# osheraz/IsaacGymInsertion

Hardware: AMD Instinct MI355X
Metric: PPO update steps/sec (4096 envs x 32 horizon) (higher is better)
Workload: dtype f32; 1 GPU; teacher PPO update, MLP actor-critic 404,501 params, 4096 envs x 32 horizon per GPU, 8 mini-epochs x 8 minibatches of 16384 (BASELINE configs[1]); envs_per_gpu=4096, horizon=32, optimizer_steps_per_update=64, parallelism=dp1, grad_allreduce=none

## Files before the change

isaacgyminsertion_amd/csrc/rowblock.h:

```cpp
#pragma once
#include <type_traits>

#include "dma_util.h"
#include "gemm_f32.h"

namespace igi {

constexpr int RB_KO = 128;
constexpr int RB_S = 64;
constexpr int RB_BR = 64;
constexpr int RB_Z_FLOATS = RB_BR * RB_KO;
constexpr int RB_X_FLOATS = RB_BR * RB_S;
constexpr int RB_STAGE = RB_Z_FLOATS + RB_X_FLOATS;
constexpr int RB_EPLD = 32 + 4;
constexpr int RB_PARK = 4 * 32 * RB_EPLD;
constexpr int RB_WPLD = RB_S + 4;
constexpr int RB_DLT = 64 + 4;
constexpr int RB_LATZ = 64 * 8 + 8 * 128 + 4 * 256 + 16 * RB_DLT;
constexpr int RB_LDS_FLOATS = 2 * RB_STAGE + RB_PARK;
constexpr int RB_LDS_FLOATS_LATZ = RB_LDS_FLOATS + RB_LATZ;
constexpr int RB_THREADS = 512;
static_assert(4 * 32 * RB_WPLD <= RB_STAGE, "the final weight-gradient tiles park in stage 0");
static_assert(2 * (32 * 66 + 32) <= RB_PARK, "the LOWX exchange uses the parking slices");

struct RbLevelArgs {
  const float* dZ = nullptr; int ldz = 0; long long sZ = 0;
  const float* W = nullptr; int ldw = 0; long long sW = 0;
  const float* X = nullptr; int ldx = 0; long long sX = 0;
  float* dX = nullptr; int lddx = 0; long long sdX = 0;
  float* dWp = nullptr; int ldwp = 0; long long sWpart = 0, sWnet = 0;
  float* dBp = nullptr; long long sBpart = 0, sBnet = 0;
  int rows = 0, IN = 0, nets = 1;
  int nslices = 0, ranges = 0, nblocks = 0;
  const float* lx_X = nullptr; int lx_ld = 0;
  float* lx_W = nullptr; int lx_ldw = 0; long long lx_sPart = 0;
  float* lx_B = nullptr; long long lx_bsPart = 0;
  const float* lz_parts = nullptr; int lz_tiles = 0; long long lz_tstride = 0;
  const float* lz_lat = nullptr; int lz_ldlat = 0;
  const float* lz_W3 = nullptr;
  float* lz_rec = nullptr; long long lz_srec = 0;
};

static inline int rb_level_ranges(int rows, int IN, int nets) {
  const int nslices = IN / RB_S, nblocks = rows / RB_BR;
  int r = 256 / (nets * nslices);
  if (r > nblocks) r = nblocks;
  return r < 1 ? 1 : r;
}

static inline bool rb_level_shape_ok(long long rows, int KO, int IN, int nets) {
  return KO == RB_KO && IN >= RB_S && (IN % RB_S) == 0 && IN <= 1024 && rows >= 4 * RB_BR && (rows % RB_BR) == 0 &&
         rows < (1 << 24) && nets >= 1 && nets <= 2 && !bf16_mode();
}

template <int MODE, int NETS>
__global__ __launch_bounds__(RB_THREADS) void k_rb_level(const RbLevelArgs a) {
  constexpr bool LOWX = MODE == 2 || MODE == 3, LATZ = MODE == 3;
  extern __shared__ __attribute__((aligned(1024))) float smem[];
  const int tid = threadIdx.x, lane = tid & 63, wave = __builtin_amdgcn_readfirstlane(tid >> 6);
  const int l31 = lane & 31, h = lane >> 5;

  const int total_ranges = NETS * a.ranges;
  int slice, gr;
  {
    const int bid = blockIdx.x;
    if ((total_ranges & 7) == 0) {
      const int x = bid & 7, p = bid >> 3;
      const int q = p / a.nslices;
      slice = p - q * a.nslices;
      gr = x * (total_ranges >> 3) + q;
    } else {
      gr = bid / a.nslices;
      slice = bid - gr * a.nslices;
    }
  }
  slice = __builtin_amdgcn_readfirstlane(slice);
  gr = __builtin_amdgcn_readfirstlane(gr);
  const int net = NETS == 1 ? 0 : __builtin_amdgcn_readfirstlane(gr / a.ranges), range = gr - net * a.ranges;
  const int b0 = __builtin_amdgcn_readfirstlane((int)((long long)range * a.nblocks / a.ranges));
  const int b1 = __builtin_amdgcn_readfirstlane((int)((long long)(range + 1) * a.nblocks / a.ranges));
  const int nb = b1 - b0;
  const int c0 = slice * RB_S;
  const float* dZ = a.dZ + net * a.sZ + (long long)b0 * RB_BR * a.ldz;
  const float* X = a.X + net * a.sX + (long long)b0 * RB_BR * a.ldx + c0;
  float* dX = a.dX + net * a.sdX + (long long)b0 * RB_BR * a.lddx + c0;
  const float* W = a.W + net * a.sW + c0;

  const bool dgrad_role = wave < 4;
  const int w4 = wave & 3;

  float* dlb = smem + 2 * RB_STAGE + RB_PARK;
  float* w3s = dlb + 64 * 8;
  float* lzx = w3s + 8 * 128;
  float* dlt = lzx + 4 * 256;
  typedef float f32x4m __attribute__((ext_vector_type(4)));
  f32x4m acc3[2] = {{0.f, 0.f, 0.f, 0.f}, {0.f, 0.f, 0.f, 0.f}};
  auto latz_head = [&](const float* zs_c, auto wg_c) __attribute__((always_inline)) {
    constexpr bool WG = decltype(wg_c)::value;
    float* zs = const_cast<float*>(zs_c);
    if constexpr (WG) {
      const int n = lane & 15, q = lane >> 4;
      const f32x4 av = *reinterpret_cast<const f32x4*>(dlt + n * RB_DLT + 16 * w4 + 4 * q);
#pragma unroll
      for (int t = 0; t < 4; ++t) {
        const int rr = 4 * q + t;
        const float* yr = zs + (16 * w4 + rr) * RB_KO + (n & 3);
#pragma unroll
        for (int jt = 0; jt < 2; ++jt) {
          const float bv = yr[4 * ((8 * slice + 4 * jt + (n >> 2)) ^ rr)];
          acc3[jt] = __builtin_amdgcn_mfma_f32_16x16x4f32(av[t], bv, acc3[jt], 0, 0, 0);
        }
      }
    }
    asm volatile("s_waitcnt lgkmcnt(0)" ::: "memory");
    __builtin_amdgcn_s_barrier();
    asm volatile("" ::: "memory");
    {
      const int cg = tid & 31, rg = tid >> 5;
      f32x4 wv[8];
#pragma unroll
      for (int k = 0; k < 8; ++k) wv[k] = *reinterpret_cast<const f32x4*>(w3s + k * 128 + 4 * cg);
      float* zp0 = zs + rg * RB_KO + 4 * (cg ^ rg);
#pragma unroll
      for (int i = 0; i < 4; ++i) {
        const int row = rg + 16 * i;
        const f32x4 d0 = *reinterpret_cast<const f32x4*>(dlb + row * 8), d1 = *reinterpret_cast<const f32x4*>(dlb + row * 8 + 4);
        f32x4* zp = reinterpret_cast<f32x4*>(zp0 + 16 * i * RB_KO);
        const f32x4 y = *zp;
        f32x4 sacc = {0.f, 0.f, 0.f, 0.f};
#pragma unroll
        for (int k = 0; k < 8; ++k) {
          const float dk = k < 4 ? d0[k & 3] : d1[k & 3];
#pragma unroll
          for (int j = 0; j < 4; ++j) sacc[j] = fmaf(dk, wv[k][j], sacc[j]);
        }
        f32x4 o;
#pragma unroll
        for (int j = 0; j < 4; ++j) o[j] = sacc[j] * (1.0f - y[j] * y[j]);
        *zp = o;
      }
    }
    asm volatile("s_waitcnt lgkmcnt(0)" ::: "memory");
    __builtin_amdgcn_s_barrier();
    asm volatile("" ::: "memory");
  };

  if (dgrad_role) {
    const int rt = w4 >> 1, ct = w4 & 1;
    __builtin_amdgcn_s_barrier();
    asm volatile("" ::: "memory");
    float wf[64];
    int zq[16];
    {
      const float* wp = smem + RB_STAGE + 4 * h * RB_S + 32 * ct + l31;
#pragma unroll
      for (int c = 0; c < 16; ++c)
#pragma unroll
        for (int j = 0; j < 4; ++j) wf[4 * c + j] = wp[(8 * c + j) * RB_S];
      const int m = 32 * rt + l31;
#pragma unroll
      for (int c = 0; c < 16; ++c) zq[c] = m * RB_KO + 4 * ((2 * c + h) ^ (m & 15));
      asm volatile("s_waitcnt lgkmcnt(0)" ::: "memory");
    }
    __builtin_amdgcn_s_barrier();
    asm volatile("" ::: "memory");
    float* park = smem + 2 * RB_STAGE + w4 * (32 * RB_EPLD);
    const int prow = lane >> 3, pc4 = lane & 7;
    unsigned lo = 4u * ((unsigned)prow * (unsigned)a.lddx + 4u * (unsigned)pc4);
    f32x16 acc_prev;
    float xv_prev[16];
#pragma unroll
    for (int r = 0; r < 16; ++r) { acc_prev[r] = 0.f; xv_prev[r] = 0.f; }
    f32x16 lxacc[2];
    float lxb = 0.f, pb0[16], pb1[16];
#pragma unroll
    for (int r = 0; r < 16; ++r) { lxacc[0][r] = 0.f; lxacc[1][r] = 0.f; pb0[r] = 0.f; pb1[r] = 0.f; }
    const float* lxbase = LOWX ? a.lx_X + ((long long)b0 * RB_BR + 32 * rt) * a.lx_ld : nullptr;
    unsigned lxo = 4u * ((unsigned)(4 * h) * (unsigned)a.lx_ld + (unsigned)l31);
    auto lx_load = [&](int bp, int r) {
      const char* q = reinterpret_cast<const char*>(uniform_ptr(lxbase + ((long long)bp * RB_BR + (r & 3) + 8 * (r >> 2)) * a.lx_ld));
      asm volatile("" : "+v"(lxo));
      pb0[r] = *reinterpret_cast<const float*>(q + lxo);
      pb1[r] = *reinterpret_cast<const float*>(q + lxo + 128);
    };
    float vprev[16];
#pragma unroll
    for (int r = 0; r < 16; ++r) vprev[r] = 0.f;
    auto epi_elem = [&](int bp, int r) {
      const float v = LOWX ? vprev[r] : acc_prev[r] * (1.0f - xv_prev[r] * xv_prev[r]);
      if (LOWX) {
        lxb += v;
        lxacc[0] = __builtin_amdgcn_mfma_f32_32x32x2f32(v, pb0[r], lxacc[0], 0, 0, 0);
        lxacc[1] = __builtin_amdgcn_mfma_f32_32x32x2f32(v, pb1[r], lxacc[1], 0, 0, 0);
      } else {
        park[((r & 3) + 8 * (r >> 2) + 4 * h) * RB_EPLD + l31] = v;
      }
    };
    f32x4 pv;
    auto epi_read = [&](int it) { pv = *reinterpret_cast<const f32x4*>(park + (8 * it + prow) * RB_EPLD + 4 * pc4); };
    auto epi_store = [&](int bp, int it) {
      char* ob = reinterpret_cast<char*>(dX + ((long long)bp * RB_BR + 32 * rt) * a.lddx + 32 * ct);
      asm volatile("" : "+v"(lo));
      *reinterpret_cast<f32x4*>(ob + (size_t)it * 8 * a.lddx * 4 + lo) = pv;
    };
    auto block = [&](int b, auto stg) {
      constexpr int S = decltype(stg)::value;
      if (b > 0) {
        __builtin_amdgcn_s_barrier();
        asm volatile("" ::: "memory");
      }
      const float* zs = smem + S * RB_STAGE;
      const float* xs = zs + RB_Z_FLOATS;
      if constexpr (LATZ) latz_head(zs, std::false_type{});
      const float* xc = xs + (32 * rt + 4 * h) * RB_S + 32 * ct + l31;
      float xv[16];
      if (!LOWX) {
#pragma unroll
        for (int r = 0; r < 16; ++r) xv[r] = xc[((r & 3) + 8 * (r >> 2)) * RB_S];
      }
      f32x16 acc;
#pragma unroll
      for (int r = 0; r < 16; ++r) acc[r] = 0.f;
      f32x4 fa[2];
      const int zrow = (32 * rt + l31) * RB_KO, zsw = (32 * rt + l31) & 15;
      auto zoffs = [&](int c) { return LOWX ? zrow + 4 * ((2 * c + h) ^ zsw) : zq[c]; };
      fa[0] = *reinterpret_cast<const f32x4*>(zs + zoffs(0));
      const bool epi = b > 0;
      if (LOWX && epi) { lx_load(b - 1, 0); lx_load(b - 1, 1); }
#pragma unroll
      for (int c = 0; c < 16; ++c) {
        if (c < 15) fa[(c + 1) & 1] = *reinterpret_cast<const f32x4*>(zs + zoffs(c + 1));
        if (epi && MODE == 0 && c >= 9 && c < 13) epi_read(c - 9);
        __builtin_amdgcn_sched_barrier(0);
#pragma unroll
        for (int j = 0; j < 4; ++j)
          acc = __builtin_amdgcn_mfma_f32_32x32x2f32(fa[c & 1][j], wf[4 * c + j], acc, 0, 0, 0);
        if (epi) {
          if (LOWX) { if (c + 2 < 16) lx_load(b - 1, c + 2); epi_elem(b - 1, c); }
          else if (c < 8) { epi_elem(b - 1, 2 * c); epi_elem(b - 1, 2 * c + 1); }
          else if (c >= 9 && c < 13) epi_store(b - 1, c - 9);
        }
        __builtin_amdgcn_sched_barrier(0);
      }
      if (LOWX) {
#pragma unroll
        for (int r = 0; r < 16; ++r) xv[r] = xc[((r & 3) + 8 * (r >> 2)) * RB_S];
#pragma unroll
        for (int r = 0; r < 16; ++r) vprev[r] = acc[r] * (1.0f - xv[r] * xv[r]);
      } else {
        acc_prev = acc;
#pragma unroll
        for (int r = 0; r < 16; ++r) xv_prev[r] = xv[r];
      }
    };
    int b = 0;
    for (; b + 2 <= nb; b += 2) {
      block(b, std::integral_constant<int, 0>{});
      block(b + 1, std::integral_constant<int, 1>{});
    }
    if (b < nb) block(b, std::integral_constant<int, 0>{});
    __syncthreads();
    if constexpr (LATZ) {
      float* rec = a.lz_rec + (long long)range * a.lz_srec;
      float s3 = 0.f;
#pragma unroll
      for (int g = 0; g < 4; ++g) s3 += lzx[g * 256 + tid];
      rec[(tid >> 5) * 128 + 32 * slice + (tid & 31)] = s3;
      if (slice == 0 && tid < 8) {
        float sdb = 0.f;
        for (int j = 0; j < 32; ++j) sdb += dlb[tid + 8 * j];
        rec[8 * 128 + tid] = sdb;
      }
    }
    if (LOWX) { lx_load(nb - 1, 0); lx_load(nb - 1, 1); }
#pragma unroll
    for (int r = 0; r < 16; ++r) {
      if (LOWX && r + 2 < 16) lx_load(nb - 1, r + 2);
      epi_elem(nb - 1, r);
    }
    if (MODE == 0) {
#pragma unroll
      for (int it = 0; it < 4; ++it) { epi_read(it); epi_store(nb - 1, it); }
    }
    if (LOWX) {
      constexpr int XLD = 64 + 2;
      float* ex = smem + 2 * RB_STAGE + ct * (32 * XLD + 32);
      const float bsum2 = lxb + __shfl_xor(lxb, 32, 64);
      if (rt == 1) {
#pragma unroll
        for (int n = 0; n < 2; ++n)
#pragma unroll
          for (int r = 0; r < 16; ++r) ex[((r & 3) + 8 * (r >> 2) + 4 * h) * XLD + 32 * n + l31] = lxacc[n][r];
        if (h == 0) ex[32 * XLD + l31] = bsum2;
      }
      __syncthreads();
      if (rt == 0) {
        float* wout = a.lx_W + range * a.lx_sPart + (long long)(c0 + 32 * ct) * a.lx_ldw;
#pragma unroll
        for (int n = 0; n < 2; ++n)
#pragma unroll
          for (int r = 0; r < 16; ++r) {
            const int c = (r & 3) + 8 * (r >> 2) + 4 * h;
            wout[(long long)c * a.lx_ldw + 32 * n + l31] = lxacc[n][r] + ex[c * XLD + 32 * n + l31];
          }
        if (h == 0) a.lx_B[range * a.lx_bsPart + c0 + 32 * ct + l31] = bsum2 + ex[32 * XLD + l31];
      }
    }
    return;
  }

  const int zr0 = 2 * w4 + (lane >> 5);
  unsigned zoff[2];
#pragma unroll
  for (int par = 0; par < 2; ++par)
    zoff[par] = 4u * ((unsigned)zr0 * (unsigned)a.ldz + 4u * (unsigned)((lane & 31) ^ ((zr0 + 8 * par) & 15)));
  unsigned xoff = 4u * ((unsigned)(4 * w4 + (lane >> 4)) * (unsigned)a.ldx + 4u * (unsigned)(lane & 15));
  auto issue = [&](int b, auto stg) {
    float* st = smem + decltype(stg)::value * RB_STAGE;
    const char* zb = reinterpret_cast<const char*>(uniform_ptr(dZ + (long long)b * RB_BR * a.ldz));
    const char* xb = reinterpret_cast<const char*>(uniform_ptr(X + (long long)b * RB_BR * a.ldx));
#pragma unroll
    for (int q = 0; q < 8; ++q) {
      asm volatile("" : "+v"(zoff[q & 1]));
      dma16(reinterpret_cast<const float*>(zb + (size_t)q * 8 * a.ldz * 4 + zoff[q & 1]), st + 256 * (w4 + 4 * q));
    }
#pragma unroll
    for (int q = 0; q < 4; ++q) {
      asm volatile("" : "+v"(xoff));
      dma16(reinterpret_cast<const float*>(xb + (size_t)q * 16 * a.ldx * 4 + xoff), st + RB_Z_FLOATS + 256 * (w4 + 4 * q));
    }
  };
  issue(0, std::integral_constant<int, 0>{});
  {
    const unsigned woff = 4u * ((unsigned)(4 * w4 + (lane >> 4)) * (unsigned)a.ldw + 4u * (unsigned)(lane & 15));
    const char* wb = reinterpret_cast<const char*>(uniform_ptr(W));
#pragma unroll
    for (int q = 0; q < 8; ++q)
      dma16(reinterpret_cast<const float*>(wb + (size_t)q * 16 * a.ldw * 4 + woff), smem + RB_STAGE + 256 * (w4 + 4 * q));
  }
  const int wt = tid - 256;
  float lzp[2][8], lzl[2] = {0.f, 0.f};
  float dbacc = 0.f;
#pragma unroll
  for (int i = 0; i < 2; ++i)
#pragma unroll
    for (int t = 0; t < 8; ++t) lzp[i][t] = 0.f;
  auto lz_fetch = [&](int b) __attribute__((always_inline)) {
#pragma unroll
    for (int i = 0; i < 2; ++i) {
      const int pr = wt + 256 * i;
      const long long grow = (long long)(b0 + b) * RB_BR + (pr >> 3);
      const float* pp = a.lz_parts + grow * 8 + (pr & 7);
#pragma unroll
      for (int t = 0; t < 8; ++t) lzp[i][t] = t < a.lz_tiles ? pp[(long long)t * a.lz_tstride] : 0.f;
      lzl[i] = a.lz_lat[grow * a.lz_ldlat + (pr & 7)];
    }
  };
  auto lz_publish = [&]() __attribute__((always_inline)) {
#pragma unroll
    for (int i = 0; i < 2; ++i) {
      float acc_ = 0.f;
#pragma unroll
      for (int t = 0; t < 8; ++t)
        if (t < a.lz_tiles) acc_ += lzp[i][t];
      const float dl = acc_ * (1.0f - lzl[i] * lzl[i]);
      dlb[wt + 256 * i] = dl;
      dlt[((wt + 256 * i) & 7) * RB_DLT + ((wt + 256 * i) >> 3)] = dl;
      dbacc += dl;
    }
  };
  if constexpr (LATZ) {
    for (int e = wt; e < 8 * 128; e += 256) w3s[e] = a.lz_W3[e];
    for (int e = wt; e < 8 * RB_DLT; e += 256) dlt[8 * RB_DLT + e] = 0.f;
    lz_fetch(0);
    lz_publish();
  }
  const int ot = w4;
  f32x16 accw[2];
  float bsum = 0.f;
  const bool do_bias = (slice == 0) && (a.dBp != nullptr);
#pragma unroll
  for (int r = 0; r < 16; ++r) { accw[0][r] = 0.f; accw[1][r] = 0.f; }
  int za[2][4];
  {
    const int o = 32 * ot + l31;
#pragma unroll
    for (int par = 0; par < 2; ++par)
#pragma unroll
      for (int j = 0; j < 4; ++j) {
        const int r = 8 * par + 4 * h + j;
        za[par][j] = (4 * h + j) * RB_KO + 4 * ((o >> 2) ^ r) + (o & 3);
      }
  }
  asm volatile("s_waitcnt vmcnt(0)" ::: "memory");
  asm volatile("s_waitcnt lgkmcnt(0)" ::: "memory");
  __builtin_amdgcn_s_barrier();
  __builtin_amdgcn_s_barrier();
  asm volatile("" ::: "memory");
  {
    auto block = [&](int b, auto stg, auto bias_c) __attribute__((always_inline)) {
      constexpr int S = decltype(stg)::value;
      constexpr bool BIAS = decltype(bias_c)::value;
      if (b > 0) {
        if constexpr (LATZ) lz_publish();
        asm volatile("s_waitcnt vmcnt(0)" ::: "memory");
        asm volatile("s_waitcnt lgkmcnt(0)" ::: "memory");
        __builtin_amdgcn_s_barrier();
        asm volatile("" ::: "memory");
      }
      const float* zs = smem + S * RB_STAGE;
      if constexpr (LATZ) {
        latz_head(zs, std::true_type{});
        if (b + 1 < nb) lz_fetch(b + 1);
      }
      const float* xb_ = zs + RB_Z_FLOATS + 4 * h * RB_S + l31;
      float fa[2][4], fb0[2][4], fb1[2][4];
      auto load = [&](int c, float (&A)[4], float (&B0)[4], float (&B1)[4]) {
#pragma unroll
        for (int j = 0; j < 4; ++j) {
          A[j] = zs[8 * c * RB_KO + za[c & 1][j]];
          B0[j] = xb_[(8 * c + j) * RB_S];
          B1[j] = xb_[(8 * c + j) * RB_S + 32];
        }
      };
      load(0, fa[0], fb0[0], fb1[0]);
      if (b + 1 < nb) issue(b + 1, std::integral_constant<int, 1 - S>{});
#pragma unroll
      for (int c = 0; c < 8; ++c) {
        if (c < 7) load(c + 1, fa[(c + 1) & 1], fb0[(c + 1) & 1], fb1[(c + 1) & 1]);
        __builtin_amdgcn_sched_barrier(0);
        if constexpr (BIAS) {
#pragma unroll
          for (int j = 0; j < 4; ++j) bsum += fa[c & 1][j];
        }
#pragma unroll
        for (int j = 0; j < 4; ++j) {
          accw[0] = __builtin_amdgcn_mfma_f32_32x32x2f32(fa[c & 1][j], fb0[c & 1][j], accw[0], 0, 0, 0);
          accw[1] = __builtin_amdgcn_mfma_f32_32x32x2f32(fa[c & 1][j], fb1[c & 1][j], accw[1], 0, 0, 0);
        }
        __builtin_amdgcn_sched_barrier(0);
      }
    };
    auto run = [&](auto bias_c) {
      int b = 0;
      for (; b + 2 <= nb; b += 2) {
        block(b, std::integral_constant<int, 0>{}, bias_c);
        block(b + 1, std::integral_constant<int, 1>{}, bias_c);
      }
      if (b < nb) block(b, std::integral_constant<int, 0>{}, bias_c);
    };
    if (do_bias) run(std::true_type{}); else run(std::false_type{});
  }

  if constexpr (LATZ) {
    if (lane < 32) {
      const int n = lane & 15, q = lane >> 4;
#pragma unroll
      for (int jt = 0; jt < 2; ++jt)
#pragma unroll
        for (int r = 0; r < 4; ++r) lzx[w4 * 256 + (4 * q + r) * 32 + 16 * jt + n] = acc3[jt][r];
    }
    dlb[wt] = dbacc;
  }
  __syncthreads();
  float* wp = smem + ot * (32 * RB_WPLD);
#pragma unroll
  for (int n = 0; n < 2; ++n)
#pragma unroll
    for (int r = 0; r < 16; ++r)
      wp[((r & 3) + 8 * (r >> 2) + 4 * h) * RB_WPLD + 32 * n + l31] = accw[n][r];
  asm volatile("s_waitcnt lgkmcnt(0)" ::: "memory");
  float* out = a.dWp + range * a.sWpart + net * a.sWnet + (long long)(32 * ot) * a.ldwp + c0;
  const int prow = lane >> 4, pc4 = lane & 15;
#pragma unroll
  for (int it = 0; it < 8; ++it) {
    const f32x4 v = *reinterpret_cast<const f32x4*>(wp + (4 * it + prow) * RB_WPLD + 4 * pc4);
    *reinterpret_cast<f32x4*>(out + (long long)(4 * it + prow) * a.ldwp + 4 * pc4) = v;
  }
  if (do_bias) {
    const float other = __shfl_xor(bsum, 32, 64);
    if (h == 0) a.dBp[range * a.sBpart + net * a.sBnet + 32 * ot + l31] = bsum + other;
  }
  if (LOWX) __syncthreads();
}

static hipError_t rb_level_backward(RbLevelArgs a, hipStream_t s, int prof_class) {
  if (!rb_level_shape_ok(a.rows, RB_KO, a.IN, a.nets)) return hipErrorNotSupported;
  if (!aligned16(a.dZ) || !aligned16(a.X) || (!a.lx_W && (!a.dX || !aligned16(a.dX))) || !aligned16(a.dWp) || (a.ldz & 3) || (a.ldx & 3) ||
      (a.lddx & 3) || (a.ldwp & 3) || (a.sZ & 3) || (a.sX & 3) || (a.sdX & 3) || (a.sWpart & 3) || (a.sWnet & 3) ||
      a.ldz < RB_KO || a.ldx < a.IN || a.lddx < a.IN || a.ldwp < a.IN || a.ldw < a.IN ||
      !aligned16(a.W) || (a.ldw & 3) || (a.sW & 3) ||
      (long long)RB_BR * a.ldz * 4 >= (1LL << 31) || (long long)RB_BR * a.ldx * 4 >= (1LL << 31))
    return hipErrorNotSupported;
  a.nslices = a.IN / RB_S;
  a.nblocks = a.rows / RB_BR;
  if (a.ranges < 1 || a.ranges > a.nblocks) return hipErrorInvalidValue;
  const bool lowx = a.lx_W != nullptr;
  if (lowx && (a.nets != 1 || !a.lx_X || !a.lx_B || a.lx_ld < 64 || a.lx_ldw < 64)) return hipErrorInvalidValue;
  const bool latz = a.lz_parts != nullptr;
  if (latz && (!lowx || !a.lz_lat || !a.lz_W3 || !a.lz_rec || a.lz_tiles < 1 || a.lz_tiles > 8 || a.lz_srec < 8 * 128 + 8 ||
               a.lz_ldlat < 8 || a.ldz != RB_KO))
    return hipErrorInvalidValue;
  static bool attr = false;
  if (!attr) {
    const void* ks[3] = {(const void*)k_rb_level<0, 1>, (const void*)k_rb_level<0, 2>, (const void*)k_rb_level<2, 1>};
    for (const void* k : ks) {
      hipError_t e = hipFuncSetAttribute(k, hipFuncAttributeMaxDynamicSharedMemorySize, (int)(sizeof(float) * RB_LDS_FLOATS));
      if (e != hipSuccess) return e;
    }
    hipError_t e = hipFuncSetAttribute((const void*)k_rb_level<3, 1>, hipFuncAttributeMaxDynamicSharedMemorySize,
                                       (int)(sizeof(float) * RB_LDS_FLOATS_LATZ));
    if (e != hipSuccess) return e;
    attr = true;
  }
  const double fl = 4.0 * a.nets * (double)a.rows * RB_KO * a.IN + (lowx ? 2.0 * (double)a.rows * a.IN * 64 : 0.0) +
                    (latz ? 4.0 * (double)a.rows * RB_KO * 8 : 0.0);
  const double by = 4.0 * a.nets * ((double)a.rows * (RB_KO + 2.0 * a.IN) + (double)RB_KO * a.IN * (1 + a.ranges));
  ProfScope ps(prof_class, s, fl, by);
  const dim3 grid(a.nets * a.ranges * a.nslices);
  const size_t shm = sizeof(float) * RB_LDS_FLOATS;
  if (latz) IGI_LAUNCH((k_rb_level<3, 1>), grid, dim3(RB_THREADS), sizeof(float) * RB_LDS_FLOATS_LATZ, s, a);
  else if (lowx) IGI_LAUNCH((k_rb_level<2, 1>), grid, dim3(RB_THREADS), shm, s, a);
  else if (a.nets == 1) IGI_LAUNCH((k_rb_level<0, 1>), grid, dim3(RB_THREADS), shm, s, a);
  else IGI_LAUNCH((k_rb_level<0, 2>), grid, dim3(RB_THREADS), shm, s, a);
  return hipGetLastError();
}

}
```

Before: 40.21 updates/s.

## Deepen LOWX prefetch with explicit vmcnt waits and MFMA-based latent head

Replaces compiler-scheduled LOWX global loads with inline-asm loads issued several rows ahead, paired with explicit vmcnt waits, to hide more global-memory latency behind the MFMA loop. The latent head's scalar FMA mat-vec over an LDS copy of W3 becomes a 32x32x2 MFMA with W3 held in registers, which removes the W3 LDS staging. The block loop is specialized so the first block skips the epilogue at compile time. Hand-written waitcnt counts are fragile and could be wrong if the compiler reorders other memory ops, and holding W3 in registers adds VGPR pressure.

After: 40.32 updates/s (median of 2 runs). No clear change (+0.3%).

```diff
diff --git a/isaacgyminsertion_amd/csrc/rowblock.h b/isaacgyminsertion_amd/csrc/rowblock.h
--- a/isaacgyminsertion_amd/csrc/rowblock.h
+++ b/isaacgyminsertion_amd/csrc/rowblock.h
@@ -16,7 +16,9 @@
 constexpr int RB_PARK = 4 * 32 * RB_EPLD;
 constexpr int RB_WPLD = RB_S + 4;
 constexpr int RB_DLT = 64 + 4;
-constexpr int RB_LATZ = 64 * 8 + 8 * 128 + 4 * 256 + 16 * RB_DLT;
+constexpr int RB_LATZ = 64 * 8 + 4 * 256 + 16 * RB_DLT;
+constexpr int RB_LX_AHEAD = 4;
+static_assert(RB_LX_AHEAD >= 1 && RB_LX_AHEAD <= 8, "lx_wait counts up to 2 * 8 younger requests");
 constexpr int RB_LDS_FLOATS = 2 * RB_STAGE + RB_PARK;
 constexpr int RB_LDS_FLOATS_LATZ = RB_LDS_FLOATS + RB_LATZ;
 constexpr int RB_THREADS = 512;
@@ -90,9 +92,13 @@
   const int w4 = wave & 3;
 
   float* dlb = smem + 2 * RB_STAGE + RB_PARK;
-  float* w3s = dlb + 64 * 8;
-  float* lzx = w3s + 8 * 128;
+  float* lzx = dlb + 64 * 8;
   float* dlt = lzx + 4 * 256;
+  float w3r[4] = {0.f, 0.f, 0.f, 0.f};
+  if constexpr (LATZ) {
+#pragma unroll
+    for (int p = 0; p < 4; ++p) w3r[p] = a.lz_W3[(2 * p + h) * 128 + 32 * (wave & 3) + l31];
+  }
   typedef float f32x4m __attribute__((ext_vector_type(4)));
   f32x4m acc3[2] = {{0.f, 0.f, 0.f, 0.f}, {0.f, 0.f, 0.f, 0.f}};
   auto latz_head = [&](const float* zs_c, auto wg_c) __attribute__((always_inline)) {
@@ -116,29 +122,24 @@
     __builtin_amdgcn_s_barrier();
     asm volatile("" ::: "memory");
     {
-      const int cg = tid & 31, rg = tid >> 5;
-      f32x4 wv[8];
-#pragma unroll
-      for (int k = 0; k < 8; ++k) wv[k] = *reinterpret_cast<const f32x4*>(w3s + k * 128 + 4 * cg);
-      float* zp0 = zs + rg * RB_KO + 4 * (cg ^ rg);
-#pragma unroll
-      for (int i = 0; i < 4; ++i) {
-        const int row = rg + 16 * i;
-        const f32x4 d0 = *reinterpret_cast<const f32x4*>(dlb + row * 8), d1 = *reinterpret_cast<const f32x4*>(dlb + row * 8 + 4);
-        f32x4* zp = reinterpret_cast<f32x4*>(zp0 + 16 * i * RB_KO);
-        const f32x4 y = *zp;
-        f32x4 sacc = {0.f, 0.f, 0.f, 0.f};
-#pragma unroll
-        for (int k = 0; k < 8; ++k) {
-          const float dk = k < 4 ? d0[k & 3] : d1[k & 3];
-#pragma unroll
-          for (int j = 0; j < 4; ++j) sacc[j] = fmaf(dk, wv[k][j], sacc[j]);
-        }
-        f32x4 o;
-#pragma unroll
-        for (int j = 0; j < 4; ++j) o[j] = sacc[j] * (1.0f - y[j] * y[j]);
-        *zp = o;
-      }
+      const int rt8 = wave >> 2, ct8 = wave & 3;
+      const float* ap = dlt + h * RB_DLT + 32 * rt8 + l31;
+      f32x16 zacc;
+#pragma unroll
+      for (int r = 0; r < 16; ++r) zacc[r] = 0.f;
+#pragma unroll
+      for (int p = 0; p < 4; ++p) zacc = __builtin_amdgcn_mfma_f32_32x32x2f32(ap[2 * p * RB_DLT], w3r[p], zacc, 0, 0, 0);
+      float* zp0 = zs + (32 * rt8 + 4 * h) * RB_KO + (l31 & 3);
+      const int cu = 8 * ct8 + (l31 >> 2);
+      auto zoff8 = [&](int r) {
+        const int rr = (r & 3) + 8 * (r >> 2);
+        return rr * RB_KO + 4 * (cu ^ ((rr & 15) + 4 * h));
+      };
+      float y[16];
+#pragma unroll
+      for (int r = 0; r < 16; ++r) y[r] = zp0[zoff8(r)];
+#pragma unroll
+      for (int r = 0; r < 16; ++r) zp0[zoff8(r)] = zacc[r] * (1.0f - y[r] * y[r]);
     }
     asm volatile("s_waitcnt lgkmcnt(0)" ::: "memory");
     __builtin_amdgcn_s_barrier();
@@ -176,12 +177,19 @@
 #pragma unroll
     for (int r = 0; r < 16; ++r) { lxacc[0][r] = 0.f; lxacc[1][r] = 0.f; pb0[r] = 0.f; pb1[r] = 0.f; }
     const float* lxbase = LOWX ? a.lx_X + ((long long)b0 * RB_BR + 32 * rt) * a.lx_ld : nullptr;
-    unsigned lxo = 4u * ((unsigned)(4 * h) * (unsigned)a.lx_ld + (unsigned)l31);
-    auto lx_load = [&](int bp, int r) {
-      const char* q = reinterpret_cast<const char*>(uniform_ptr(lxbase + ((long long)bp * RB_BR + (r & 3) + 8 * (r >> 2)) * a.lx_ld));
-      asm volatile("" : "+v"(lxo));
-      pb0[r] = *reinterpret_cast<const float*>(q + lxo);
-      pb1[r] = *reinterpret_cast<const float*>(q + lxo + 128);
+    const unsigned lxo = 4u * ((unsigned)(4 * h) * (unsigned)a.lx_ld + (unsigned)l31);
+    auto lx_load = [&](int bp, int r) __attribute__((always_inline)) {
+      const float* q = uniform_ptr(lxbase + ((long long)bp * RB_BR + (r & 3) + 8 * (r >> 2)) * a.lx_ld);
+      asm volatile("s_nop 4\n\tglobal_load_dword %0, %2, %3\n\tglobal_load_dword %1, %2, %3 offset:128"
+                   : "=&v"(pb0[r]), "=&v"(pb1[r]) : "v"(lxo), "s"(q));
+    };
+    auto lx_wait = [&](int r) __attribute__((always_inline)) {
+      const int young = 2 * (15 - r < RB_LX_AHEAD ? 15 - r : RB_LX_AHEAD);
+#define RB_LX_WAIT(N) case N: asm volatile("s_waitcnt vmcnt(" #N ")" : "+v"(pb0[r]), "+v"(pb1[r])); break;
+      switch (young) {
+        RB_LX_WAIT(0) RB_LX_WAIT(2) RB_LX_WAIT(4) RB_LX_WAIT(6) RB_LX_WAIT(8) RB_LX_WAIT(10) RB_LX_WAIT(12) RB_LX_WAIT(14) RB_LX_WAIT(16)
+      }
+#undef RB_LX_WAIT
     };
     float vprev[16];
 #pragma unroll
@@ -203,9 +211,10 @@
       asm volatile("" : "+v"(lo));
       *reinterpret_cast<f32x4*>(ob + (size_t)it * 8 * a.lddx * 4 + lo) = pv;
     };
-    auto block = [&](int b, auto stg) {
-      constexpr int S = decltype(stg)::value;
-      if (b > 0) {
+    auto block = [&](int b, auto stg, auto epi_c) __attribute__((always_inline)) {
+      constexpr int S = decltype(stg)::value, EPI = decltype(epi_c)::value;
+      const bool epi = EPI < 0 ? b > 0 : EPI > 0;
+      if (epi) {
         __builtin_amdgcn_s_barrier();
         asm volatile("" ::: "memory");
       }
@@ -225,8 +234,10 @@
       const int zrow = (32 * rt + l31) * RB_KO, zsw = (32 * rt + l31) & 15;
       auto zoffs = [&](int c) { return LOWX ? zrow + 4 * ((2 * c + h) ^ zsw) : zq[c]; };
       fa[0] = *reinterpret_cast<const f32x4*>(zs + zoffs(0));
-      const bool epi = b > 0;
-      if (LOWX && epi) { lx_load(b - 1, 0); lx_load(b - 1, 1); }
+      if (LOWX && epi) {
+#pragma unroll
+        for (int r = 0; r < RB_LX_AHEAD; ++r) lx_load(b - 1, r);
+      }
 #pragma unroll
       for (int c = 0; c < 16; ++c) {
         if (c < 15) fa[(c + 1) & 1] = *reinterpret_cast<const f32x4*>(zs + zoffs(c + 1));
@@ -236,7 +247,7 @@
         for (int j = 0; j < 4; ++j)
           acc = __builtin_amdgcn_mfma_f32_32x32x2f32(fa[c & 1][j], wf[4 * c + j], acc, 0, 0, 0);
         if (epi) {
-          if (LOWX) { if (c + 2 < 16) lx_load(b - 1, c + 2); epi_elem(b - 1, c); }
+          if (LOWX) { if (c + RB_LX_AHEAD < 16) lx_load(b - 1, c + RB_LX_AHEAD); lx_wait(c); epi_elem(b - 1, c); }
           else if (c < 8) { epi_elem(b - 1, 2 * c); epi_elem(b - 1, 2 * c + 1); }
           else if (c >= 9 && c < 13) epi_store(b - 1, c - 9);
         }
@@ -253,12 +264,25 @@
         for (int r = 0; r < 16; ++r) xv_prev[r] = xv[r];
       }
     };
-    int b = 0;
-    for (; b + 2 <= nb; b += 2) {
-      block(b, std::integral_constant<int, 0>{});
-      block(b + 1, std::integral_constant<int, 1>{});
-    }
-    if (b < nb) block(b, std::integral_constant<int, 0>{});
+    if constexpr (LOWX) {
+      constexpr std::integral_constant<int, 0> first{};
+      constexpr std::integral_constant<int, 1> later{};
+      block(0, std::integral_constant<int, 0>{}, first);
+      int b = 1;
+      for (; b + 2 <= nb; b += 2) {
+        block(b, std::integral_constant<int, 1>{}, later);
+        block(b + 1, std::integral_constant<int, 0>{}, later);
+      }
+      if (b < nb) block(b, std::integral_constant<int, 1>{}, later);
+    } else {
+      constexpr std::integral_constant<int, -1> any{};
+      int b = 0;
+      for (; b + 2 <= nb; b += 2) {
+        block(b, std::integral_constant<int, 0>{}, any);
+        block(b + 1, std::integral_constant<int, 1>{}, any);
+      }
+      if (b < nb) block(b, std::integral_constant<int, 0>{}, any);
+    }
     __syncthreads();
     if constexpr (LATZ) {
       float* rec = a.lz_rec + (long long)range * a.lz_srec;
@@ -272,10 +296,16 @@
         rec[8 * 128 + tid] = sdb;
       }
     }
-    if (LOWX) { lx_load(nb - 1, 0); lx_load(nb - 1, 1); }
+    if (LOWX) {
+#pragma unroll
+      for (int r = 0; r < RB_LX_AHEAD; ++r) lx_load(nb - 1, r);
+    }
 #pragma unroll
     for (int r = 0; r < 16; ++r) {
-      if (LOWX && r + 2 < 16) lx_load(nb - 1, r + 2);
+      if (LOWX) {
+        if (r + RB_LX_AHEAD < 16) lx_load(nb - 1, r + RB_LX_AHEAD);
+        lx_wait(r);
+      }
       epi_elem(nb - 1, r);
     }
     if (MODE == 0) {
@@ -370,7 +400,6 @@
     }
   };
   if constexpr (LATZ) {
-    for (int e = wt; e < 8 * 128; e += 256) w3s[e] = a.lz_W3[e];
     for (int e = wt; e < 8 * RB_DLT; e += 256) dlt[8 * RB_DLT + e] = 0.f;
     lz_fetch(0);
     lz_publish();
```
